# beyzoskaya/HiC-GNN

Hardware: AMD Instinct MI355X
Metric: training steps/sec (GATNetSelectiveResidualsUpdated, fwd+loss+bwd+Adam) (higher is better)
Workload: dtype fp32; 1 GPU; synth-20000; n_nodes=20000, nnz_with_self_loops=4019956, d=512, heads=2, loss=mse, parallelism=single, gemm=fp32 MFMA

## Files before the change

### hic-gnn_amd/csrc/gemm.hip

```cpp
#include <algorithm>
#include <cstdlib>

#include "reduce.hpp"

namespace hicgat {

typedef float f32x16 __attribute__((ext_vector_type(16)));

constexpr int GK = 16;

constexpr int kOcc64 = 6, kOcc128 = 1;

template <int BM, int BN, bool A_KM, bool B_KM, bool VEC, bool DB, bool CS = false>
__device__ __forceinline__ void gemm_tile(const float *__restrict__ A, int64_t lda,
                                          const float *__restrict__ B, int64_t ldb,
                                          float *__restrict__ C, int64_t ldc, int M, int N,
                                          int K, int kchunk, const float *__restrict__ bias,
                                          float *__restrict__ slab, int64_t slab_stride, int accumulate,
                                          float *__restrict__ csum, int bx, int by, int bz,
                                          float *__restrict__ crelu = nullptr, int64_t ldr = 0) {
  static_assert(!CS || A_KM, "column sums of A need the K-major (weight-gradient) layout");
  constexpr int WM = BM / 2, WN = BN / 2;
  constexpr int TM = WM / 32, TN = WN / 32;
  constexpr int AE = VEC ? BM * GK / 1024 : BM * GK / 256;
// ... 166 lines not shown
                                                   float *__restrict__ csum) {
  gemm_tile<BM, BN, A_KM, B_KM, VEC, DB, CS>(A, lda, B, ldb, C, ldc, M, N, K, kchunk, bias, slab, slab_stride, accumulate,
                                             csum, blockIdx.x, blockIdx.y, blockIdx.z);
}

__global__ void colsum_zero_kernel(float *out, int N, int accumulate) {
  const int n = blockIdx.x * 256 + threadIdx.x;
  if (n < N && !accumulate) out[n] = 0.f;
}

int gemm_wgrad_ring_launch(const float *A, int64_t lda, const float *B, int64_t ldb, int M, int N, int K, int kchunk,
                           int splits, float *slab, int64_t slab_stride, hipStream_t s);

template <int BM, int BN, bool AK, bool BK_>
static int launch(const float *A, int64_t lda, const float *B, int64_t ldb, float *C, int64_t ldc, int M, int N,
                  int K, int splits, const float *bias, float *slab, int acc, hipStream_t s, float *csum = nullptr,
                  bool ring = false) {
  const int kchunk = ((K + splits - 1) / splits + GK - 1) / GK * GK;
  const dim3 grid((M + BM - 1) / BM, (N + BN - 1) / BN, splits);
  const bool a_ok = AK ? (M % 4 == 0 && lda % 4 == 0) : (K % 4 == 0 && lda % 4 == 0);
  const bool b_ok = BK_ ? (N % 4 == 0 && ldb % 4 == 0) : (K % 4 == 0 && ldb % 4 == 0);
  const bool al = ((reinterpret_cast<uintptr_t>(A) | reinterpret_cast<uintptr_t>(B)) & 15) == 0;
  const bool cs = AK && csum != nullptr;
  const int64_t stride = (int64_t)M * N + (cs ? M : 0);
  float *sl = splits > 1 ? slab : nullptr;
  float *cdst = cs ? (sl ? slab + (int64_t)M * N : csum) : nullptr;
#define HICGAT_GEMM_GO(V, D, C_)                                                                            \
  hipLaunchKernelGGL((gemm_kernel<BM, BN, AK, BK_, V, D, C_>), grid, dim3(256), 0, s, A, lda, B, ldb, C, ldc, M, N, \
                     K, kchunk, bias, sl, stride, acc, cdst)
  int ring_rc = HICGAT_EUNSUPPORTED;
  if (ring && AK && BK_ && BM == 128 && BN == 128 && sl && !cs)
    ring_rc = gemm_wgrad_ring_launch(A, lda, B, ldb, M, N, K, kchunk, splits, sl, stride, s);
  if (ring_rc == HICGAT_OK) {
  } else if (ring_rc != HICGAT_EUNSUPPORTED) {
    return ring_rc;
  } else if (a_ok && b_ok && al) {
    constexpr bool db = !AK && BK_;
    if (cs) HICGAT_GEMM_GO(true, db, AK);
    else HICGAT_GEMM_GO(true, db, false);
  } else {
    if (cs) HICGAT_GEMM_GO(false, false, AK);
    else HICGAT_GEMM_GO(false, false, false);
  }
#undef HICGAT_GEMM_GO
  HICGAT_CHECK_LAUNCH();
  if (splits > 1) {
    const ColOut o{C, ldc, N, nullptr, bias, acc, cs ? csum : nullptr, (int64_t)M * N};
    return colsum_wide_launch(slab, stride, splits, stride, o, s);
  }
  return HICGAT_OK;
}

int gemm_tall_launch(bool b_kmajor, const float *A, int64_t lda, const float *B, int64_t ldb, float *C, int64_t ldc,
                     int M, int N, int K, const float *bias, int accumulate, hipStream_t s);

static int64_t tall_min_tiles() { return 192; }

template <bool AK, bool BK_>
static int dispatch(const float *A, int64_t lda, const float *B, int64_t ldb, float *C, int64_t ldc, int M, int N,
                    int K, int splits, const float *bias, float *slab, int acc, int impl, hipStream_t s) {
  if (!AK && splits == 1 && M >= 1024 &&
      (int64_t)((M + 159) / 160) * (N / 128) >= tall_min_tiles()) {
    const int rc = gemm_tall_launch(BK_, A, lda, B, ldb, C, ldc, M, N, K, bias, acc, s);
    if (rc != HICGAT_EUNSUPPORTED) return rc;
  }
  if (M >= 128 && N >= 128 && M <= 1024) {
    const bool ring = AK && BK_ && impl == HICGAT_GEMM_AUTO && splits > 1 && M % 128 == 0 && N % 128 == 0 &&
                      N <= 1024 && lda % 4 == 0 && ldb % 4 == 0;
    return launch<128, 128, AK, BK_>(A, lda, B, ldb, C, ldc, M, N, K, splits, bias, slab, acc, s, nullptr, ring);
  }
  if (N >= 128) return launch<64, 128, AK, BK_>(A, lda, B, ldb, C, ldc, M, N, K, splits, bias, slab, acc, s);
  return launch<64, 64, AK, BK_>(A, lda, B, ldb, C, ldc, M, N, K, splits, bias, slab, acc, s);
}

constexpr int kMaxWJobs = 16, kMaxCJobs = 32, kGroupTile = 128;
constexpr int64_t WEIGHTED_LG1_ROWS = 1024;
#ifndef HICGAT_COLSUM_SHORT
#define HICGAT_COLSUM_SHORT 16
#endif
constexpr int64_t kColsumShortRows = HICGAT_COLSUM_SHORT;
constexpr int kWeightedLg = 1;
template <int KMAX>
__device__ __forceinline__ int find_job(const int (&start)[KMAX], int n, int b) {
  int q = 0;
#pragma unroll
  for (int k = 1; k < KMAX; ++k) q += (k < n && b >= start[k]) ? 1 : 0;
  return q;
}
struct WJob {
  const float *dy;
  const float *x;
  float *dw;
  float *db;
  float *slab;
  int64_t ldy, ldx, lddw;
  int M, N, K, kchunk, tm, tn, wg0, accumulate, vec;
};
struct WJobs {
  int start[kMaxWJobs];
  WJob j[kMaxWJobs];
  int n;
};
__global__ __launch_bounds__(256, kOcc128) void wgrad_grouped_kernel(const WJobs jobs) {
  const int q = find_job(jobs.start, jobs.n, (int)blockIdx.x);
  const WJob &J = jobs.j[q];
  const int local = blockIdx.x - J.wg0, per = J.tm * J.tn;
  const int bz = local / per, rem = local - bz * per, bx = rem % J.tm, by = rem / J.tm;
  const int64_t stride = (int64_t)J.M * J.N + J.M;
  float *cs = J.db ? (J.slab ? J.slab + (int64_t)J.M * J.N : J.db) : nullptr;
  if (J.vec)
    gemm_tile<kGroupTile, kGroupTile, true, true, true, false, true>(J.dy, J.ldy, J.x, J.ldx, J.dw, J.lddw, J.M, J.N,
                                                                     J.K, J.kchunk, nullptr, J.slab, stride,
                                                                     J.accumulate, cs, bx, by, bz);
  else
    gemm_tile<kGroupTile, kGroupTile, true, true, false, false, true>(J.dy, J.ldy, J.x, J.ldx, J.dw, J.lddw, J.M, J.N,
                                                                      J.K, J.kchunk, nullptr, J.slab, stride,
// ... 301 lines not shown
    J.wg0 = wg;
    wj.start[wj.n - 1] = wg;
    wg += J.tm * J.tn * sp;
    if (sp > 1) {
      const int64_t stride = (int64_t)a.M * a.N + a.M;
      int rc = add_col(J.slab, stride, sp, (int64_t)a.M * a.N, a.dw, a.accumulate);
      if (rc != HICGAT_OK) return rc;
      if (a.db && (rc = add_col(J.slab + (int64_t)a.M * a.N, stride, sp, a.M, a.db, a.accumulate)) != HICGAT_OK)
        return rc;
    }
  }
  for (int i = 0; i < nc; ++i) {
    if (c[i].rows < 0 || c[i].cols < 0 || (c[i].cols > 0 && !c[i].dst) || (c[i].rows > 0 && !c[i].src))
      return HICGAT_EINVAL;
    const int rc = add_col(c[i].src, c[i].ld, c[i].rows, c[i].cols, c[i].dst, c[i].accumulate, c[i].wt, c[i].ldw,
                           c[i].segs, c[i].ldd);
    if (rc != HICGAT_OK) return rc;
  }
  if (wg > 0) {
    hipLaunchKernelGGL(wgrad_grouped_kernel, dim3(wg), dim3(256), 0, s, wj);
    HICGAT_CHECK_LAUNCH();
  }
  if (blk > 0) {
    hipLaunchKernelGGL(colsum_grouped_kernel, dim3(blk), dim3(256), 0, s, cj);
    HICGAT_CHECK_LAUNCH();
  }
  return HICGAT_OK;
}

extern "C" size_t hicgat_gemm_workspace_bytes(int M, int N, int splits) {
  return splits > 1 ? (size_t)splits * M * N * sizeof(float) : 0;
}

extern "C" int hicgat_gemm(int a_kmajor, int b_kmajor, int M, int N, int K, const float *A, int64_t lda,
                           const float *B, int64_t ldb, const float *bias, float *C, int64_t ldc,
                           int accumulate, int splits, int impl, void *workspace, size_t workspace_bytes,
                           hicgat_stream_t stream) {
  if (impl == HICGAT_GEMM_X3) return HICGAT_EUNSUPPORTED;
  if (impl != HICGAT_GEMM_AUTO && impl != HICGAT_GEMM_F32) return HICGAT_EINVAL;
  if (M < 0 || N < 0 || K < 0 || splits < 1) return HICGAT_EINVAL;
  if (M == 0 || N == 0) return HICGAT_OK;
  if (!A || !B || !C) return HICGAT_EINVAL;
  if (splits > 1 && (!workspace || workspace_bytes < hicgat_gemm_workspace_bytes(M, N, splits)))
    return HICGAT_EINVAL;
  hipStream_t s = (hipStream_t)stream;
  float *slab = static_cast<float *>(workspace);
  const int i = impl;
  if (!a_kmajor && !b_kmajor) return dispatch<false, false>(A, lda, B, ldb, C, ldc, M, N, K, splits, bias, slab, accumulate, i, s);
  if (!a_kmajor && b_kmajor) return dispatch<false, true>(A, lda, B, ldb, C, ldc, M, N, K, splits, bias, slab, accumulate, i, s);
  if (a_kmajor && !b_kmajor) return dispatch<true, false>(A, lda, B, ldb, C, ldc, M, N, K, splits, bias, slab, accumulate, i, s);
  return dispatch<true, true>(A, lda, B, ldb, C, ldc, M, N, K, splits, bias, slab, accumulate, i, s);
}

extern "C" size_t hicgat_gemm_wgrad_workspace_bytes(int M, int N, int splits) {
  return splits > 1 ? (size_t)splits * ((size_t)M * N + M) * sizeof(float) : 0;
}

extern "C" int hicgat_gemm_wgrad(int M, int N, int K, const float *dY, int64_t ldy, const float *X, int64_t ldx,
                                 float *dW, int64_t lddw, float *db, int accumulate, int splits, void *workspace,
                                 size_t workspace_bytes, hicgat_stream_t stream) {
  if (M < 0 || N < 0 || K < 0 || splits < 1 || lddw < N) return HICGAT_EINVAL;
  if (M == 0 || N == 0) return HICGAT_OK;
  if (!dY || !X || !dW) return HICGAT_EINVAL;
  if (splits > 1 && (!workspace || workspace_bytes < hicgat_gemm_wgrad_workspace_bytes(M, N, splits)))
    return HICGAT_EINVAL;
  hipStream_t s = (hipStream_t)stream;
  float *slab = static_cast<float *>(workspace);
  if (M >= 128 && N >= 128 && M <= 1024)
    return launch<128, 128, true, true>(dY, ldy, X, ldx, dW, lddw, M, N, K, splits, nullptr, slab, accumulate, s, db);
  if (N >= 128) return launch<64, 128, true, true>(dY, ldy, X, ldx, dW, lddw, M, N, K, splits, nullptr, slab, accumulate, s, db);
  return launch<64, 64, true, true>(dY, ldy, X, ldx, dW, lddw, M, N, K, splits, nullptr, slab, accumulate, s, db);
}

extern "C" size_t hicgat_colsum_workspace_bytes(int K, int N) { return colsum_workspace_bytes(K, N); }

extern "C" int hicgat_colsum(const float *A, int64_t lda, int K, int N, float *out, int accumulate, void *workspace,
                             size_t workspace_bytes, hicgat_stream_t stream) {
  if (K < 0 || N < 0) return HICGAT_EINVAL;
  if (N == 0) return HICGAT_OK;
  if (!out || (K > 0 && !A)) return HICGAT_EINVAL;
  const size_t need = colsum_workspace_bytes(K, N);
  if (need > 0 && (!workspace || workspace_bytes < need)) return HICGAT_EINVAL;
  hipStream_t s = (hipStream_t)stream;
  const ColOut o{out, 0, N, nullptr, nullptr, accumulate};
  if (K == 0) {
    hipLaunchKernelGGL(colsum_zero_kernel, dim3((N + 255) / 256), dim3(256), 0, s, out, N, accumulate);
    HICGAT_CHECK_LAUNCH();
    return HICGAT_OK;
  }
  return colsum_launch(A, lda, K, N, o, static_cast<float *>(workspace), s);
}
```

### hic-gnn_amd/csrc/gemm_tall.hip

```cpp
#include "common.hpp"

namespace hicgat {

namespace {

constexpr int TBM = 160, TBN = 128, TBK = 16, TSLOTS = 3;
constexpr int TA_F = TBM * TBK;
constexpr int TB_F = TBN * TBK;
constexpr int TSTAGE_F = TA_F + TB_F;
constexpr size_t kTallLds = (size_t)TSLOTS * TSTAGE_F * sizeof(float);
constexpr int TA_PIECES = TA_F * 4 / 1024;
constexpr int TB_PIECES = TB_F * 4 / 1024;

typedef float f32x16 __attribute__((ext_vector_type(16)));
typedef float f4v __attribute__((ext_vector_type(4)));

__device__ __forceinline__ int kc_slot(int r, int g) { return g ^ ((r >> 2) & 3); }

template <bool BKC>
__device__ __forceinline__ void tall_issue(float *stage, const float *__restrict__ A, int64_t lda, int m0, int M,
                                           const float *__restrict__ B, int64_t ldb, int n0, int k0, int w,
                                           int lane) {
  for (int p = w; p < TA_PIECES; p += 4) {
    const int r = 16 * p + (lane >> 2), s = lane & 3;
    const int gm = min(m0 + r, M - 1);
    const float *src = A + (size_t)gm * lda + k0 + 4 * kc_slot(r, s);
    __builtin_amdgcn_global_load_lds(src, stage + p * 256, 16, 0, 0);
  }
  float *bs = stage + TA_F;
  for (int p = w; p < TB_PIECES; p += 4) {
    const float *src;
    if (BKC) {
      const int r = 16 * p + (lane >> 2), s = lane & 3;
      src = B + (size_t)(n0 + r) * ldb + k0 + 4 * kc_slot(r, s);
    } else {
      const int t = 2 * p + (lane >> 5);
      src = B + (size_t)(k0 + t) * ldb + n0 + (lane & 31) * 4;
    }
    __builtin_amdgcn_global_load_lds(src, bs + p * 256, 16, 0, 0);
  }
}

}

template <bool BKC>
__global__ __launch_bounds__(256, 2) void gemm_tall_kernel(const float *__restrict__ A, int64_t lda,
                                                          const float *__restrict__ B, int64_t ldb,
                                                          float *__restrict__ C, int64_t ldc, int M, int N, int K,
                                                          const float *__restrict__ bias, int accumulate) {
  extern __shared__ __attribute__((aligned(16))) float lds[];
  const int lane = threadIdx.x & 63, w = wave_in_block();
  const int li = lane & 31, lk = lane >> 5;
  const int ntn = N / TBN;
  const int tile = xcd_remap(blockIdx.x, gridDim.x);
  const int m0 = (tile / ntn) * TBM, n0 = (tile % ntn) * TBN;
  const int S = K / TBK;
  f32x16 acc[5];
#pragma unroll
  for (int t = 0; t < 5; ++t)
#pragma unroll
    for (int r = 0; r < 16; ++r) acc[t][r] = 0.f;

  tall_issue<BKC>(lds, A, lda, m0, M, B, ldb, n0, 0, w, lane);
  if (S > 1) tall_issue<BKC>(lds + TSTAGE_F, A, lda, m0, M, B, ldb, n0, TBK, w, lane);
  const bool w_more = w < TA_PIECES - 8;

  const int bcol = 32 * w + li;
  const uint32_t lds_base = (uint32_t)(uintptr_t)lds;
  const uint32_t a_row = (uint32_t)(li * TBK * 4);
  const uint32_t b_row = (uint32_t)(TA_F * 4) + (BKC ? (uint32_t)(bcol * TBK * 4) : (uint32_t)(bcol * 4));

  for (int s = 0; s < S; ++s) {
    if (s + 1 < S) {
      if (w_more) asm volatile("s_waitcnt vmcnt(5)" ::: "memory");
      else asm volatile("s_waitcnt vmcnt(4)" ::: "memory");
    } else {
      asm volatile("s_waitcnt vmcnt(0)" ::: "memory");
    }
    asm volatile("s_waitcnt lgkmcnt(0)" ::: "memory");
    __builtin_amdgcn_s_barrier();
    asm volatile("" ::: "memory");
    if (s + 2 < S)
      tall_issue<BKC>(lds + ((s + 2) % TSLOTS) * TSTAGE_F, A, lda, m0, M, B, ldb, n0, (s + 2) * TBK, w, lane);
    const uint32_t st = lds_base + (uint32_t)((s % TSLOTS) * TSTAGE_F * 4);
#pragma unroll
    for (int p = 0; p < TBK / 8; ++p) {
      const int g = 2 * p + lk;
      const uint32_t aa = st + a_row + (uint32_t)(kc_slot(li, g) * 16);
      f4v a0, a1, a2, a3, a4;
      float bk[4];
      if (BKC) {
        const uint32_t ba = st + b_row + (uint32_t)(kc_slot(bcol, g) * 16);
        f4v b;
        asm volatile(
            "ds_read_b128 %0, %6\n\tds_read_b128 %1, %6 offset:2048\n\tds_read_b128 %2, %6 offset:4096\n\t"
            "ds_read_b128 %3, %6 offset:6144\n\tds_read_b128 %4, %6 offset:8192\n\tds_read_b128 %5, %7\n\t"
            "s_waitcnt lgkmcnt(0)"
            : "=&v"(a0), "=&v"(a1), "=&v"(a2), "=&v"(a3), "=&v"(a4), "=&v"(b)
            : "v"(aa), "v"(ba)
            : "memory");
        bk[0] = b.x;
        bk[1] = b.y;
        bk[2] = b.z;
        bk[3] = b.w;
      } else {
        const uint32_t ba = st + b_row + (uint32_t)((8 * p + 4 * lk) * TBN * 4);
        asm volatile(
            "ds_read_b128 %0, %9\n\tds_read_b128 %1, %9 offset:2048\n\tds_read_b128 %2, %9 offset:4096\n\t"
            "ds_read_b128 %3, %9 offset:6144\n\tds_read_b128 %4, %9 offset:8192\n\t"
            "ds_read_b32 %5, %10\n\tds_read_b32 %6, %10 offset:512\n\tds_read_b32 %7, %10 offset:1024\n\t"
            "ds_read_b32 %8, %10 offset:1536\n\ts_waitcnt lgkmcnt(0)"
            : "=&v"(a0), "=&v"(a1), "=&v"(a2), "=&v"(a3), "=&v"(a4), "=&v"(bk[0]), "=&v"(bk[1]), "=&v"(bk[2]), "=&v"(bk[3])
            : "v"(aa), "v"(ba)
            : "memory");
      }
      const f4v a[5] = {a0, a1, a2, a3, a4};
#pragma unroll
      for (int c = 0; c < 4; ++c)
#pragma unroll
        for (int t = 0; t < 5; ++t) acc[t] = __builtin_amdgcn_mfma_f32_32x32x2f32(a[t][c], bk[c], acc[t], 0, 0, 0);
    }
  }

  const int gn = n0 + bcol;
  const float bb = bias ? bias[gn] : 0.f;
#pragma unroll
  for (int t = 0; t < 5; ++t) {
    float old[16];
#pragma unroll
    for (int r = 0; r < 16; ++r) old[r] = 0.f;
    if (accumulate) {
#pragma unroll
      for (int r = 0; r < 16; ++r) {
        const int gm = min(m0 + 32 * t + (r & 3) + 8 * (r >> 2) + 4 * lk, M - 1);
        old[r] = C[(size_t)gm * ldc + gn];
      }
    }
#pragma unroll
    for (int r = 0; r < 16; ++r) {
      const int gm = m0 + 32 * t + (r & 3) + 8 * (r >> 2) + 4 * lk;
      if (gm < M) C[(size_t)gm * ldc + gn] = acc[t][r] + bb + old[r];
    }
  }
}

int gemm_tall_launch(bool b_kmajor, const float *A, int64_t lda, const float *B, int64_t ldb, float *C, int64_t ldc,
                     int M, int N, int K, const float *bias, int accumulate, hipStream_t s) {
  const bool al = ((reinterpret_cast<uintptr_t>(A) | reinterpret_cast<uintptr_t>(B)) & 15) == 0;
  if (!al || M < TBM || N % TBN || K % TBK || K < TBK || lda % 4 || ldb % 4) return HICGAT_EUNSUPPORTED;
  const int64_t tiles = (int64_t)((M + TBM - 1) / TBM) * (N / TBN);
  if (tiles > 0x7fffffff) return HICGAT_EUNSUPPORTED;
  if (b_kmajor)
    hipLaunchKernelGGL(gemm_tall_kernel<false>, dim3((unsigned)tiles), dim3(256), kTallLds, s, A, lda, B, ldb, C, ldc, M,
                       N, K, bias, accumulate);
  else
    hipLaunchKernelGGL(gemm_tall_kernel<true>, dim3((unsigned)tiles), dim3(256), kTallLds, s, A, lda, B, ldb, C, ldc, M,
                       N, K, bias, accumulate);
  HICGAT_CHECK_LAUNCH();
  return HICGAT_OK;
}

}
```

### hic-gnn_amd/hicgat/_lib.py

```python
import ctypes
import os

import torch

from . import streams as _streams

_HERE = os.path.dirname(os.path.abspath(__file__))
LIB_PATH = os.environ.get("HICGAT_LIB", os.path.join(_HERE, "libhicgat.so"))

c_int, c_i64, c_f, c_d, c_sz, c_p = (ctypes.c_int, ctypes.c_int64, ctypes.c_float, ctypes.c_double,
                                     ctypes.c_size_t, ctypes.c_void_p)
c_u64, c_u32 = ctypes.c_uint64, ctypes.c_uint32


class WgradJob(ctypes.Structure):
    _fields_ = [("dy", c_p), ("ldy", c_i64), ("x", c_p), ("ldx", c_i64), ("dw", c_p), ("lddw", c_i64), ("db", c_p),
                ("M", c_int), ("N", c_int), ("K", c_int), ("accumulate", c_int)]


class ColsumJob(ctypes.Structure):
    _fields_ = [("src", c_p), ("ld", c_i64), ("rows", c_i64), ("cols", c_i64), ("dst", c_p), ("accumulate", c_int),
                ("wt", c_p), ("ldw", c_i64), ("segs", c_int), ("ldd", c_i64)]


# ... 23 lines not shown
                                       c_i64, c_p, c_i64, c_p, c_p, c_f, c_p, c_p, c_int, c_p]),
    "hicgat_gat_agg_drop_fwd": (c_int, [c_p, c_p, c_int, c_int, c_int, c_int, c_int, c_int, c_p, c_p, c_p,
                                        c_p, c_f, c_int, c_p, c_p, c_p, c_d, c_u64, c_p, c_i64, c_u32, c_p]),
    "hicgat_gat_agg_drop_bwd_src": (c_int, [c_p, c_p, c_int, c_int, c_int, c_int, c_int, c_p, c_p, c_p, c_p,
                                            c_i64, c_p, c_i64, c_p, c_p, c_f, c_p, c_p, c_int, c_d, c_u64, c_p,
                                            c_i64, c_u32, c_p]),
    "hicgat_gat_attn_mask": (c_int, [c_p, c_p, c_int, c_int, c_d, c_u64, c_p, c_i64, c_u32, c_p, c_p]),
    "hicgat_gat_agg_fwd_tiled": (c_int, [c_p, c_p, c_p, c_p, c_p, c_p, c_p, c_int, c_int, c_int, c_int, c_int,
                                         c_int, c_p, c_p, c_p, c_p, c_f, c_int, c_p, c_p, c_p, c_int, c_p, c_sz,
                                         c_p]),
    "hicgat_gat_agg_bwd_src_tiled": (c_int, [c_p, c_p, c_p, c_p, c_p, c_int, c_int, c_int, c_int, c_int, c_int,
                                             c_p, c_p, c_p, c_p, c_i64, c_p, c_i64, c_p, c_p, c_f, c_p, c_p, c_int,
                                             c_p, c_sz, c_p]),
    "hicgat_gat_tiled_workspace_bytes": (c_sz, [c_int, c_int]),
    "hicgat_gat_param_grad": (c_int, [c_p, c_p, c_p, c_p, c_int, c_int, c_int, c_p, c_p, c_p, c_int, c_p,
                                      c_sz, c_p]),
    "hicgat_gat_param_grad_workspace_bytes": (c_sz, [c_int, c_int]),
    "hicgat_gat_transpose_map": (c_int, [c_p, c_p, c_int, c_p, c_p]),
    "hicgat_gat_alpha": (c_int, [c_p, c_p, c_int, c_int, c_int, c_p, c_p, c_p, c_f, c_p, c_p]),
    "hicgat_gat_alpha_bwd_dst": (c_int, [c_p, c_p, c_int, c_int, c_int, c_p, c_p, c_p, c_p, c_f, c_p, c_p, c_p]),
    "hicgat_gat_alpha_bwd_src": (c_int, [c_p, c_p, c_p, c_int, c_int, c_int, c_p, c_p, c_p, c_p, c_p, c_p, c_p, c_p,
                                         c_f, c_p, c_p, c_p, c_p]),
    "hicgat_pairdist_fwd": (c_int, [c_p, c_int, c_p, c_i64, c_p]),
    "hicgat_pairdist_bwd": (c_int, [c_p, c_p, c_int, c_i64, c_p, c_p, c_sz, c_p]),
    "hicgat_pairdist_mse_fused": (c_int, [c_p, c_p, c_int, c_i64, c_i64, c_i64, c_i64, c_i64, c_i64, c_int,
                                          c_p, c_p, c_p, c_p, c_sz, c_p]),
    "hicgat_pairdist_finalize": (c_int, [c_int, c_int, c_p, c_p, c_p]),
    "hicgat_pairdist_finalize_rows": (c_int, [c_int, c_int, c_p, c_p, c_p, c_int, c_int, c_p, c_p, c_p, c_p, c_p]),
    "hicgat_pairdist_num_tiles": (c_i64, [c_int, c_int]),
    "hicgat_pairdist_workspace_bytes": (c_sz, [c_int, c_int]),
    "hicgat_pairdist_mse_fused_support": (c_int, [c_p, c_p, c_int, c_f, c_p, c_p, c_p, c_p, c_i64, c_i64,
                                                  c_int, c_int, c_int, c_p, c_p, c_p, c_p, c_p, c_sz, c_p]),
    "hicgat_pairdist_support_workspace_bytes": (c_sz, [c_int]),
    "hicgat_xagg_vec_bytes": (c_sz, []),
    "hicgat_xagg_logits": (c_int, [c_p, c_p, c_p, c_p, c_int, c_int, c_int, c_int, c_p, c_p, c_p, c_p,
                                   c_i64, c_p, c_p, c_p, c_p, c_sz, c_p]),
    "hicgat_xagg_fwd": (c_int, [c_p, c_p, c_int, c_int, c_int, c_int, c_int, c_int, c_p, c_p, c_p, c_f, c_p, c_p,
                                c_p]),
    "hicgat_xagg_bias_relu": (c_int, [c_p, c_p, c_p, c_int, c_int, c_p]),
    "hicgat_xagg_rows_bwd": (c_int, [c_int, c_int, c_int, c_p, c_p, c_p, c_p, c_p, c_p]),
    "hicgat_xagg_edge": (c_int, [c_p, c_p, c_int, c_int, c_int, c_int, c_int, c_int, c_p, c_p, c_p, c_p, c_p, c_p,
                                 c_f, c_p, c_p]),
    "hicgat_xagg_edge_acc": (c_int, [c_p, c_p, c_int, c_int, c_int, c_int, c_int, c_int, c_p, c_p, c_p, c_p, c_p,
                                     c_p, c_f, c_p, c_p]),
    "hicgat_xagg_edge_acc_blocks": (c_int, [c_int]),
    "hicgat_xagg_slab_workspace_bytes": (c_sz, []),
    "hicgat_xagg_slab_sum": (c_int, [c_p, c_p, c_int, c_p, c_p, c_p, c_p, c_p, c_sz, c_p]),
    "hicgat_xagg_param_finish": (c_int, [c_p, c_p, c_p, c_p, c_p, c_int, c_i64, c_int, c_int, c_int, c_p, c_p,
                                         c_p, c_p]),
    "hicgat_truth_support": (c_int, [c_p, c_int, c_i64, c_f, c_p, c_p, c_p, c_p, c_p]),
    "hicgat_gemm": (c_int, [c_int, c_int, c_int, c_int, c_int, c_p, c_i64, c_p, c_i64, c_p, c_p, c_i64, c_int,
                            c_int, c_int, c_p, c_sz, c_p]),
    "hicgat_gemm_workspace_bytes": (c_sz, [c_int, c_int, c_int]),
    "hicgat_gemm_wgrad": (c_int, [c_int, c_int, c_int, c_p, c_i64, c_p, c_i64, c_p, c_i64, c_p, c_int, c_int, c_p,
                                  c_sz, c_p]),
    "hicgat_gemm_wgrad_workspace_bytes": (c_sz, [c_int, c_int, c_int]),
    "hicgat_gemm_rows_grouped_workspace_bytes": (c_sz, [c_gjobs, c_int, c_int]),
    "hicgat_gemm_rows_grouped": (c_int, [c_gjobs, c_int, c_int, c_int, c_p, c_sz, c_p]),
    "hicgat_param_grads_workspace_bytes": (c_sz, [c_wjobs, c_int, c_int]),
    "hicgat_param_grads_grouped": (c_int, [c_wjobs, c_int, c_cjobs, c_int, c_int, c_p, c_sz, c_p]),
    "hicgat_colsum": (c_int, [c_p, c_i64, c_int, c_int, c_p, c_int, c_p, c_sz, c_p]),
    "hicgat_colsum_workspace_bytes": (c_sz, [c_int, c_int]),
    "hicgat_ln_act_res_fwd": (c_int, [c_p, c_i64, c_int, c_int, c_p, c_p, c_f, c_int, c_f, c_p, c_i64, c_p, c_p, c_f,
                                      c_p, c_i64, c_p, c_p, c_p]),
    "hicgat_ln_act_res_bwd": (c_int, [c_p, c_i64, c_p, c_i64, c_int, c_int, c_p, c_p, c_p, c_int, c_f, c_p, c_i64,
                                      c_p, c_p, c_p, c_i64, c_p, c_i64, c_p, c_p, c_p, c_p, c_int, c_p, c_sz, c_p]),
    "hicgat_ln_act_res_bwd_params": (c_int, [c_int, c_p, c_p, c_p, c_p, c_int, c_p, c_sz, c_p]),
    "hicgat_ln_act_res_workspace_bytes": (c_sz, [c_int, c_int]),
    "hicgat_act_fwd": (c_int, [c_p, c_int, c_int, c_int, c_f, c_p, c_p]),
    "hicgat_act_bwd": (c_int, [c_p, c_p, c_int, c_int, c_int, c_f, c_p, c_p]),
    "hicgat_tail_pack_bytes": (c_sz, []),
    "hicgat_tail_pack": (c_int, [c_p, c_p, c_p, c_p, c_sz, c_p]),
    "hicgat_tail_fwd_fused": (c_int, [c_p, c_i64, c_int] + [c_p] * 14 + [c_f] + [c_p] * 10 + [c_p, c_p]),
    "hicgat_tail_bwd_waves": (c_int, []),
    "hicgat_tail_bwd_workspace_bytes": (c_sz, [c_int, c_int]),
    "hicgat_tail_bwd_fused": (c_int, [c_p, c_int] + [c_p] * 16 + [c_p] * 4 + [c_p, c_sz] * 3 + [c_p, c_p]),
    "hicgat_tail_fwd_fused_heads": (c_int, [c_p, c_i64, c_i64, c_p, c_p, c_p, c_p, c_int] + [c_p] * 14 + [c_f]
                                    + [c_p] * 10 + [c_p, c_p]),
    "hicgat_tail_bwd_fused_rows": (c_int, [c_p, c_int] + [c_p] * 16 + [c_p] * 3 + [c_p, c_sz] * 3
                                   + [c_int, c_p, c_p, c_p, c_p, c_p, c_p, c_p]),
    "hicgat_tail_bwd_fused_heads": (c_int, [c_p, c_int] + [c_p] * 16 + [c_p] * 3 + [c_p, c_sz] * 3
                                    + [c_int, c_p, c_p, c_p, c_p, c_p, c_p, c_p, c_p]),
    "hicgat_sage_weights": (c_int, [c_p, c_int, c_i64, c_p, c_p, c_p, c_p, c_p]),
    "hicgat_sage_agg": (c_int, [c_p, c_p, c_p, c_p, c_int, c_int, c_int, c_int, c_p, c_int, c_int, c_p, c_i64,
                                c_p]),
    "hicgat_kr_matvec": (c_int, [c_p, c_i64, c_int, c_p, c_p, c_p, c_p, c_p]),
    "hicgat_kr_scale": (c_int, [c_p, c_i64, c_int, c_p, c_p, c_i64, c_p]),
    "hicgat_n2v_walks": (c_int, [c_p, c_p, c_p, c_int, c_p, c_int, c_int, c_f, c_f, c_u64, c_p, c_p]),
    "hicgat_n2v_sgns_epoch": (c_int, [c_p, c_int, c_int, c_p, c_p, c_int, c_int, c_int, c_int, c_f, c_f, c_int,
                                      c_int, c_u64, c_int, c_p, c_p, c_p]),
    "hicgat_line_workspace_bytes": (c_sz, [c_int, c_int]),
    "hicgat_line_samples": (c_int, [c_p, c_p, c_p, c_p, c_int, c_p, c_p, c_int, c_p, c_i64, c_i64, c_int, c_int,
                                    c_u64, c_i64, c_i64, c_p, c_p, c_p, c_p]),
    "hicgat_line_train": (c_int, [c_p, c_p, c_p, c_p, c_int, c_p, c_p, c_int, c_p, c_i64, c_i64, c_int, c_int, c_int,
                                  c_u64, c_i64, c_i64, c_d, c_d, c_d, c_d, c_p, c_p, c_p, c_p, c_p, c_p, c_p, c_sz,
                                  c_p]),
    "hicgat_adam_step": (c_int, [c_p, c_p, c_p, c_p, c_i64, c_d, c_d, c_d, c_d, c_i64, c_p]),
    "hicgat_adam_step_table": (c_int, [c_p, c_p, c_p, c_p, c_i64, c_d, c_d, c_d, c_p, c_i64, c_p, c_int, c_p]),
    "hicgat_step_begin": (c_int, [c_p, c_i64, c_p, c_p]),
    "hicgat_step_begin_pack": (c_int, [c_p, c_i64, c_p, c_p, c_p, c_p, c_p, c_sz, c_p]),
    "hicgat_act_dropout_fwd": (c_int, [c_p, c_i64, c_int, c_int, c_int, c_f, c_d, c_u64, c_p, c_i64, c_u32, c_i64,
                                       c_p, c_i64, c_p]),
    "hicgat_act_dropout_bwd": (c_int, [c_p, c_i64, c_p, c_i64, c_int, c_int, c_int, c_f, c_d, c_p, c_i64, c_p]),
    "hicgat_dropout_mask": (c_int, [c_p, c_int, c_int, c_d, c_u64, c_p, c_i64, c_u32, c_i64, c_p]),
    "hicgat_dropout_advance": (c_int, [c_p, c_p]),
    "hicgat_bn_workspace_bytes": (c_sz, [c_int, c_int]),
# ... 70 lines not shown
```

### hic-gnn_amd/hicgat/kernels.py

```python
import os

import torch

from . import _lib
from .paramgrads import ColsumJob, WeightGradJob

TIMERS = None
GEMM_AUTO = 0
GEMM_F32 = 1


class _timed:
    def __init__(self, name):
        self.name = name

    def __enter__(self):
        if TIMERS is not None:
            self.e0 = torch.cuda.Event(enable_timing=True)
            self.e0.record()

    def __exit__(self, *a):
        if TIMERS is not None:
            e1 = torch.cuda.Event(enable_timing=True)
            e1.record()
# ... 324 lines not shown
    def fused_loss_support_range(self, coords, sf, n, kind, t0, t1, s0, s1, stats, loss, dcoords, cmap=None):
        ws = _lib.workspace(self.lib.hicgat_pairdist_support_workspace_bytes(n), coords.device)
        d32, d64 = (None, dcoords) if dcoords.dtype == torch.float64 else (dcoords, None)
        assert cmap is None or (cmap.dtype == torch.int32 and cmap.numel() == n)
        with _timed("pairdist_mse_fused"):
            _lib.check(self.lib.hicgat_pairdist_mse_fused_support(
                P(coords), P(cmap), n, sf.background, P(sf.rowptr), P(sf.col_buf), P(sf.val_buf), P(sf.diag), int(t0),
                int(t1), int(s0), int(s1), int(kind), P(stats), P(loss), P(d32), P(d64), P(ws), ws.numel(),
                _lib.stream(coords.device)), "hicgat_pairdist_mse_fused_support")

    def loss_finalize(self, n, kind, stats, loss, dc64=None, r0=0, r1=0, dcoords=None, reorder=None):
        if dc64 is None:
            _lib.check(self.lib.hicgat_pairdist_finalize(n, int(kind), P(stats), P(loss), _lib.stream(stats.device)),
                       "hicgat_pairdist_finalize")
            return
        assert dc64.is_contiguous() and dcoords.is_contiguous() and dc64.shape == dcoords.shape == (n, 3)
        cbuf, gidx, cglob = reorder if reorder is not None else (None, None, None)
        if reorder is not None:
            assert cbuf.is_contiguous() and cglob.shape == (n, 3) and gidx.dtype == torch.int32 and gidx.numel() == n
        _lib.check(self.lib.hicgat_pairdist_finalize_rows(n, int(kind), P(stats), P(loss), P(dc64), int(r0), int(r1),
                                                          P(dcoords), P(cbuf), P(gidx), P(cglob),
                                                          _lib.stream(stats.device)),
                   "hicgat_pairdist_finalize_rows")

    def pairdist_fwd(self, coords):
        n = coords.shape[0]
        D = torch.empty((n, n), dtype=torch.float32, device=coords.device)
        _lib.check(self.lib.hicgat_pairdist_fwd(P(coords), n, P(D), n, _lib.stream(coords.device)),
                   "hicgat_pairdist_fwd")
        return D

    def pairdist_bwd(self, coords, G):
        n = coords.shape[0]
        dc = torch.empty_like(coords)
        ws = _lib.workspace(self.lib.hicgat_pairdist_workspace_bytes(n, self.PD_SQUARE), coords.device)
        _lib.check(self.lib.hicgat_pairdist_bwd(P(coords), P(G), n, G.shape[1], P(dc), P(ws), ws.numel(),
                                                _lib.stream(coords.device)), "hicgat_pairdist_bwd")
        return dc

    def gemm(self, a_kmajor, b_kmajor, M, N, K, A, B, C, bias=None, accumulate=False, splits=None, name="gemm",
             impl=None):
        dev = C.device
        ws = None
        impl = self.gemm_impl if impl is None else impl
        if splits is None:
            splits = row_splits(M, N, K) if (not a_kmajor and impl in (GEMM_AUTO, GEMM_F32)) else 1
        if splits > 1:
            ws = _lib.workspace(self.lib.hicgat_gemm_workspace_bytes(M, N, splits), dev)
        with _timed(name):
            _lib.check(self.lib.hicgat_gemm(int(a_kmajor), int(b_kmajor), M, N, K, P(A), A.stride(0), P(B),
                                            B.stride(0), P(bias), P(C), C.stride(0), int(accumulate), int(splits),
                                            int(impl), P(ws), 0 if ws is None else ws.numel(), _lib.stream(dev)),
                       "hicgat_gemm")
        return C

    def wgrad(self, dy, x, W_out, b_out=None, accumulate=False, splits=1):
        K_, M = dy.shape
        N = x.shape[1]
        dev = W_out.device
        ws = None
        if splits > 1:
            ws = _lib.workspace(self.lib.hicgat_gemm_wgrad_workspace_bytes(M, N, splits), dev)
        with _timed("gemm_dw"):
            _lib.check(self.lib.hicgat_gemm_wgrad(M, N, K_, P(dy), dy.stride(0), P(x), x.stride(0), P(W_out),
                                                  W_out.stride(0), P(b_out), int(accumulate), int(splits), P(ws),
                                                  0 if ws is None else ws.numel(), _lib.stream(dev)),
                       "hicgat_gemm_wgrad")
        return W_out, b_out

    GROUP_WGS = int(os.environ.get("HICGAT_GROUP_WGS", "512"))
    ROWS_WGS = int(os.environ.get("HICGAT_ROWS_WGS", "512"))
    SMALL_M = 16

    def param_grads_grouped(self, wjobs, cjobs, target_wgs=None, small_m=None):
        target = self.GROUP_WGS if target_wgs is None else target_wgs
        small_m = self.SMALL_M if small_m is None else small_m
        big, cjobs = [], [ColsumJob(*j) for j in cjobs]
        for j in (WeightGradJob(*j) for j in wjobs):
            if j.dy.shape[1] < small_m:
                cjobs += [ColsumJob(j.x, j.dW[m], j.accumulate, j.dy[:, m]) for m in range(j.dy.shape[1])]
                if j.db is not None:
                    cjobs.append(ColsumJob(j.dy, j.db, j.accumulate))
            else:
                big.append(j)
        wjobs = big
        W = (_lib.WgradJob * max(1, len(wjobs)))()
        for k, (dy, x, dw, db, acc) in enumerate(wjobs):
            assert dy.stride(1) == 1 and x.stride(1) == 1 and dw.stride(1) == 1 and dy.shape[0] == x.shape[0]
            assert db is None or db.is_contiguous()
            W[k] = _lib.WgradJob(dy.data_ptr(), dy.stride(0), x.data_ptr(), x.stride(0), dw.data_ptr(), dw.stride(0),
                                 None if db is None else db.data_ptr(), dy.shape[1], x.shape[1], dy.shape[0], int(acc))
        C = (_lib.ColsumJob * max(1, len(cjobs)))()
        for k, (src, dst, acc, wt) in enumerate(cjobs):
            assert src.dim() == 2 and src.stride(1) == 1
            if dst.dim() == 2:
                assert dst.stride(1) == 1 and dst.shape[1] == src.shape[1] and 1 <= dst.shape[0] <= max(1, src.shape[0])
                segs, ldd = dst.shape[0], dst.stride(0)
            else:
                assert dst.is_contiguous() and dst.numel() == src.shape[1]
                segs, ldd = 1, 0
            assert wt is None or (wt.dim() == 1 and wt.shape[0] == src.shape[0])
            C[k] = _lib.ColsumJob(src.data_ptr(), src.stride(0), src.shape[0], src.shape[1], dst.data_ptr(), int(acc),
                                  None if wt is None else wt.data_ptr(), 0 if wt is None else wt.stride(0), segs, ldd)
        dev = (wjobs[0][0] if wjobs else cjobs[0][0]).device
        ws = _lib.workspace(self.lib.hicgat_param_grads_workspace_bytes(W, len(wjobs), target), dev)
        with _timed("param_grads_grouped"):
# ... 274 lines not shown
```

### include/hicgat.h

```cpp
#ifndef HICGAT_H
#define HICGAT_H

#include <stddef.h>
#include <stdint.h>

#ifdef __cplusplus
extern "C" {
#endif

typedef void *hicgat_stream_t;

enum { HICGAT_LOSS_MSE = 0, HICGAT_LOSS_COMBINED = 1, HICGAT_LOSS_CONTRASTIVE = 2 };

enum {
  HICGAT_OK = 0,
  HICGAT_EINVAL = -1,
  HICGAT_ELAUNCH = -2,
  HICGAT_EUNSUPPORTED = -3
};

int hicgat_version(void);
const char *hicgat_strerror(int code);

int hicgat_csr_from_dense(const double *A, int N, int64_t lda, int32_t *rowptr, int32_t *col,
// ... 86 lines not shown

int hicgat_gat_agg_fwd_tiled(const int32_t *rowptr, const int32_t *col, const int32_t *rowptr_s,
                             const int32_t *col_s, const int32_t *tptr, const int32_t *tcol,
                             const uint32_t *tmask, int ntiles, int N, int H, int C, int row_begin,
                             int row_end, const float *h, const float *a_src, const float *a_dst,
                             const float *bias, float neg_slope, int act, float *out, float *out2,
                             float *row_stats, int splits, void *workspace, size_t workspace_bytes,
                             hicgat_stream_t stream);
int hicgat_gat_agg_bwd_src_tiled(const int32_t *rowptr_s, const int32_t *col_s, const int32_t *tptr,
                                 const int32_t *tcol, const uint32_t *tmask, int ntiles, int N, int H,
                                 int C, int row_begin, int row_end, const float *h, const float *a_src,
                                 const float *a_dst, const float *row_stats, int64_t ld_stats,
                                 const float *dout, int64_t ld_dout, const float *att_src,
                                 const float *att_dst, float neg_slope, float *dh, float *da_src,
                                 int splits, void *workspace, size_t workspace_bytes,
                                 hicgat_stream_t stream);
size_t hicgat_gat_tiled_workspace_bytes(int rows, int splits);
int hicgat_gat_param_grad(const float *h, const float *dout, const float *da_src,
                          const float *row_stats, int N, int H, int C, float *datt_src,
                          float *datt_dst, float *dbias, int accumulate, void *workspace,
                          size_t workspace_bytes, hicgat_stream_t stream);
size_t hicgat_gat_param_grad_workspace_bytes(int N, int D);

int hicgat_pairdist_fwd(const float *coords, int N, float *D, int64_t ldd, hicgat_stream_t stream);
int hicgat_pairdist_bwd(const float *coords, const float *G, int N, int64_t ldg, float *dcoords,
                        void *workspace, size_t workspace_bytes, hicgat_stream_t stream);

int hicgat_pairdist_mse_fused(const float *coords, const float *T, int N, int64_t ldt, int64_t t_row0,
                              int64_t t_rows, int64_t t_col0, int64_t tile_begin, int64_t tile_end,
                              int loss_kind, double *stats, float *loss, float *dcoords, void *workspace,
                              size_t workspace_bytes, hicgat_stream_t stream);
int hicgat_pairdist_finalize(int N, int loss_kind, double *stats, float *loss, hicgat_stream_t stream);
int hicgat_pairdist_finalize_rows(int N, int loss_kind, double *stats, float *loss, const double *dc64,
                                  int row_begin, int row_end, float *dcoords, const float *cbuf,
                                  const int32_t *gidx, float *cglob, hicgat_stream_t stream);
enum { HICGAT_PD_SQUARE = 0, HICGAT_PD_TRI = 1 };
int64_t hicgat_pairdist_num_tiles(int N, int mode);
size_t hicgat_pairdist_workspace_bytes(int N, int mode);
int hicgat_pairdist_mse_fused_support(const float *coords, const int32_t *cmap, int N, float background,
                                      const int32_t *rowptr, const int32_t *col, const float *val,
                                      const float *diag, int64_t tile_begin, int64_t tile_end,
                                      int support_row_begin, int support_row_end, int loss_kind,
                                      double *stats, float *loss, float *dcoords, double *dcoords64,
                                      void *workspace, size_t workspace_bytes, hicgat_stream_t stream);
size_t hicgat_pairdist_support_workspace_bytes(int N);
int hicgat_truth_support(const float *T, int N, int64_t ldt, float background, int32_t *rowptr, int32_t *col,
                         float *val, float *diag, hicgat_stream_t stream);

enum { HICGAT_GEMM_AUTO = 0, HICGAT_GEMM_F32 = 1, HICGAT_GEMM_X3 = 2 };
int hicgat_gemm(int a_kmajor, int b_kmajor, int M, int N, int K, const float *A, int64_t lda,
                const float *B, int64_t ldb, const float *bias, float *C, int64_t ldc, int accumulate,
                int splits, int impl, void *workspace, size_t workspace_bytes, hicgat_stream_t stream);
size_t hicgat_gemm_workspace_bytes(int M, int N, int splits);
int hicgat_gemm_wgrad(int M, int N, int K, const float *dY, int64_t ldy, const float *X, int64_t ldx, float *dW,
                      int64_t lddw, float *db, int accumulate, int splits, void *workspace, size_t workspace_bytes,
                      hicgat_stream_t stream);
size_t hicgat_gemm_wgrad_workspace_bytes(int M, int N, int splits);
typedef struct hicgat_wgrad_job {
  const float *dy;
  int64_t ldy;
  const float *x;
  int64_t ldx;
  float *dw;
  int64_t lddw;
  float *db;
  int M, N, K, accumulate;
} hicgat_wgrad_job;
typedef struct hicgat_colsum_job {
  const float *src;
  int64_t ld;
  int64_t rows;
  int64_t cols;
  float *dst;
  int accumulate;
  const float *wt;
  int64_t ldw;
  int segs;
  int64_t ldd;
} hicgat_colsum_job;
size_t hicgat_param_grads_workspace_bytes(const hicgat_wgrad_job *wjobs, int nw, int target_wgs);
int hicgat_param_grads_grouped(const hicgat_wgrad_job *wjobs, int nw, const hicgat_colsum_job *cjobs, int nc,
                               int target_wgs, void *workspace, size_t workspace_bytes, hicgat_stream_t stream);
typedef struct hicgat_gemm_job {
  const float *a;
  int64_t lda;
  const float *b;
  int64_t ldb;
  float *c;
  int64_t ldc;
  float *c_relu;
  int64_t ldr;
  const float *bias;
  int M, N, K;
} hicgat_gemm_job;
size_t hicgat_gemm_rows_grouped_workspace_bytes(const hicgat_gemm_job *jobs, int n, int splits);
int hicgat_gemm_rows_grouped(const hicgat_gemm_job *jobs, int n, int b_kmajor, int splits, void *workspace,
                             size_t workspace_bytes, hicgat_stream_t stream);
int hicgat_colsum(const float *A, int64_t lda, int K, int N, float *out, int accumulate, void *workspace,
                  size_t workspace_bytes, hicgat_stream_t stream);
size_t hicgat_colsum_workspace_bytes(int K, int N);

int hicgat_ln_act_res_fwd(const float *y, int64_t ldy, int M, int W, const float *gamma, const float *beta, float eps,
                          int act, float slope, const float *res, int64_t ldr, const float *gamma2, const float *beta2,
                          float eps2, float *z, int64_t ldz, float *row_stats, float *row_stats2,
                          hicgat_stream_t stream);
int hicgat_ln_act_res_bwd(const float *dz, int64_t lddz, const float *y, int64_t ldy, int M, int W,
// ... 139 lines not shown
```

Baseline: 593.1 steps/s.

## Add software-pipelined tall GEMM kernel with interleaved async LDS loads and MFMA

Adds a new tall-GEMM kernel that rotates through a three-slot LDS ring. Each wave issues global_load_lds copies through inline asm that sets m0, and hand-scheduled ds_read_b128 fragment reads interleave with the 32x32x2 fp32 MFMAs, so global loads, LDS reads and math overlap within each K step. The old kernel is kept as the 'burst' variant and is used only when impl is F32; AUTO now takes the new path. The change also exposes a direct hicgat_gemm_tall entry point and factors out the store epilogue. The hand-written asm waitcnt and barrier scheduling is fragile: a wrong count would race on LDS. The new kernel is launched with zero dynamic LDS and uses a static shared array instead.

```diff
diff --git a/hic-gnn_amd/csrc/gemm.hip b/hic-gnn_amd/csrc/gemm.hip
--- a/hic-gnn_amd/csrc/gemm.hip
+++ b/hic-gnn_amd/csrc/gemm.hip
@@ -242,7 +242,8 @@
 }
 
 int gemm_tall_launch(bool b_kmajor, const float *A, int64_t lda, const float *B, int64_t ldb, float *C, int64_t ldc,
-                     int M, int N, int K, const float *bias, int accumulate, hipStream_t s);
+                     int M, int N, int K, const float *bias, int accumulate, bool burst,
+                     hipStream_t s);
 
 static int64_t tall_min_tiles() { return 192; }
 
@@ -251,7 +252,7 @@
                     int K, int splits, const float *bias, float *slab, int acc, int impl, hipStream_t s) {
   if (!AK && splits == 1 && M >= 1024 &&
       (int64_t)((M + 159) / 160) * (N / 128) >= tall_min_tiles()) {
-    const int rc = gemm_tall_launch(BK_, A, lda, B, ldb, C, ldc, M, N, K, bias, acc, s);
+    const int rc = gemm_tall_launch(BK_, A, lda, B, ldb, C, ldc, M, N, K, bias, acc, impl == HICGAT_GEMM_F32, s);
     if (rc != HICGAT_EUNSUPPORTED) return rc;
   }
   if (M >= 128 && N >= 128 && M <= 1024) {
@@ -659,6 +660,17 @@
   return dispatch<true, true>(A, lda, B, ldb, C, ldc, M, N, K, splits, bias, slab, accumulate, i, s);
 }
 
+extern "C" int hicgat_gemm_tall(int b_kmajor, int M, int N, int K, const float *A, int64_t lda, const float *B,
+                                int64_t ldb, const float *bias, float *C, int64_t ldc, int accumulate, int impl,
+                                hicgat_stream_t stream) {
+  if (impl != HICGAT_GEMM_AUTO && impl != HICGAT_GEMM_F32) return HICGAT_EINVAL;
+  if (M < 0 || N < 0 || K < 0 || lda < K || ldb < (b_kmajor ? N : K) || ldc < N) return HICGAT_EINVAL;
+  if (M == 0 || N == 0) return HICGAT_OK;
+  if (!A || !B || !C) return HICGAT_EINVAL;
+  return gemm_tall_launch(b_kmajor != 0, A, lda, B, ldb, C, ldc, M, N, K, bias, accumulate, impl == HICGAT_GEMM_F32,
+                          (hipStream_t)stream);
+}
+
 extern "C" size_t hicgat_gemm_wgrad_workspace_bytes(int M, int N, int splits) {
   return splits > 1 ? (size_t)splits * ((size_t)M * N + M) * sizeof(float) : 0;
 }
diff --git a/hic-gnn_amd/csrc/gemm_tall.hip b/hic-gnn_amd/csrc/gemm_tall.hip
--- a/hic-gnn_amd/csrc/gemm_tall.hip
+++ b/hic-gnn_amd/csrc/gemm_tall.hip
@@ -9,6 +9,7 @@
 constexpr int TB_F = TBN * TBK;
 constexpr int TSTAGE_F = TA_F + TB_F;
 constexpr size_t kTallLds = (size_t)TSLOTS * TSTAGE_F * sizeof(float);
+static_assert(kTallLds <= 80 * 1024, "two workgroups per CU in 160 KiB of LDS");
 constexpr int TA_PIECES = TA_F * 4 / 1024;
 constexpr int TB_PIECES = TB_F * 4 / 1024;
 
@@ -41,10 +42,41 @@
   }
 }
 
+__device__ __forceinline__ void tall_glds(const float *src, uint32_t dst) {
+  uint32_t keep;
+  asm volatile("s_mov_b32 %0, m0\n\ts_mov_b32 m0, %2\n\ts_nop 0\n\tglobal_load_lds_dwordx4 %1, off\n\ts_mov_b32 m0, %0"
+               : "=&s"(keep)
+               : "v"(src), "s"(dst)
+               : "memory");
+}
+
+__device__ __forceinline__ void tall_store(const f32x16 (&acc)[5], float *__restrict__ C, int64_t ldc, int M, int m0,
+                                           int gn, int lk, const float *__restrict__ bias, int accumulate) {
+  const float bb = bias ? bias[gn] : 0.f;
+#pragma unroll
+  for (int t = 0; t < 5; ++t) {
+    float old[16];
+#pragma unroll
+    for (int r = 0; r < 16; ++r) old[r] = 0.f;
+    if (accumulate) {
+#pragma unroll
+      for (int r = 0; r < 16; ++r) {
+        const int gm = min(m0 + 32 * t + (r & 3) + 8 * (r >> 2) + 4 * lk, M - 1);
+        old[r] = C[(size_t)gm * ldc + gn];
+      }
+    }
+#pragma unroll
+    for (int r = 0; r < 16; ++r) {
+      const int gm = m0 + 32 * t + (r & 3) + 8 * (r >> 2) + 4 * lk;
+      if (gm < M) C[(size_t)gm * ldc + gn] = acc[t][r] + bb + old[r];
+    }
+  }
+}
+
 }
 
 template <bool BKC>
-__global__ __launch_bounds__(256, 2) void gemm_tall_kernel(const float *__restrict__ A, int64_t lda,
+__global__ __launch_bounds__(256, 2) void gemm_tall_burst_kernel(const float *__restrict__ A, int64_t lda,
                                                           const float *__restrict__ B, int64_t ldb,
                                                           float *__restrict__ C, int64_t ldc, int M, int N, int K,
                                                           const float *__restrict__ bias, int accumulate) {
@@ -122,40 +154,181 @@
     }
   }
 
-  const int gn = n0 + bcol;
-  const float bb = bias ? bias[gn] : 0.f;
-#pragma unroll
-  for (int t = 0; t < 5; ++t) {
-    float old[16];
-#pragma unroll
-    for (int r = 0; r < 16; ++r) old[r] = 0.f;
-    if (accumulate) {
-#pragma unroll
-      for (int r = 0; r < 16; ++r) {
-        const int gm = min(m0 + 32 * t + (r & 3) + 8 * (r >> 2) + 4 * lk, M - 1);
-        old[r] = C[(size_t)gm * ldc + gn];
+  tall_store(acc, C, ldc, M, m0, n0 + bcol, lk, bias, accumulate);
+}
+
+template <bool BKC>
+__global__ __launch_bounds__(256, 2) void gemm_tall_kernel(const float *__restrict__ A, int64_t lda,
+                                                          const float *__restrict__ B, int64_t ldb,
+                                                          float *__restrict__ C, int64_t ldc, int M, int N, int K,
+                                                          const float *__restrict__ bias, int accumulate) {
+  static_assert(TBK == 16, "two k-group pairs per stage: one per fragment register set");
+  __shared__ __attribute__((aligned(16))) float lds[TSLOTS * TSTAGE_F];
+  const int lane = threadIdx.x & 63, w = wave_in_block();
+  const int li = lane & 31, lk = lane >> 5;
+  const int ntn = N / TBN;
+  const int tile = xcd_remap(blockIdx.x, gridDim.x);
+  const int m0 = (tile / ntn) * TBM, n0 = (tile % ntn) * TBN;
+  const int S = K / TBK;
+  f32x16 acc[5];
+#pragma unroll
+  for (int t = 0; t < 5; ++t)
+#pragma unroll
+    for (int r = 0; r < 16; ++r) acc[t][r] = 0.f;
+
+  const bool w_more = w < TA_PIECES - 8;
+  const float *pa[3], *pb[2];
+#pragma unroll
+  for (int h = 0; h < 3; ++h) {
+    const int r = 16 * (w + 4 * h) + (lane >> 2);
+    pa[h] = A + (size_t)min(m0 + r, M - 1) * lda + 4 * kc_slot(r, lane & 3);
+  }
+#pragma unroll
+  for (int h = 0; h < 2; ++h) {
+    const int p = w + 4 * h;
+    if (BKC) {
+      const int r = 16 * p + (lane >> 2);
+      pb[h] = B + (size_t)(n0 + r) * ldb + 4 * kc_slot(r, lane & 3);
+    } else {
+      pb[h] = B + (size_t)(2 * p + (lane >> 5)) * ldb + n0 + (lane & 31) * 4;
+    }
+  }
+  const int64_t b_step = BKC ? (int64_t)TBK : (int64_t)TBK * ldb;
+  const uint32_t lds_base = (uint32_t)(uintptr_t)lds;
+  auto issue = [&](int slot_, int q) {
+    const uint32_t dst = lds_base + (uint32_t)((slot_ * TSTAGE_F + (q & 1) * TA_F + (w + 4 * (q >> 1)) * 256) * 4);
+    tall_glds((q & 1) ? pb[q >> 1] : pa[q >> 1], dst);
+  };
+  auto advance = [&](int q, bool more) {
+    if (q & 1) pb[q >> 1] += more ? b_step : (int64_t)0;
+    else pa[q >> 1] += more ? TBK : 0;
+  };
+#pragma unroll
+  for (int st = 0; st < 2; ++st) {
+#pragma unroll
+    for (int q = 0; q < 4; ++q) issue(st, q);
+    if (w_more) issue(st, 4);
+#pragma unroll
+    for (int q = 0; q < 5; ++q) advance(q, st + 1 < S);
+  }
+
+  const int bcol = 32 * w + li;
+  uint32_t a_off[2], b_off[2];
+#pragma unroll
+  for (int p = 0; p < 2; ++p) {
+    a_off[p] = (uint32_t)(li * TBK * 4 + kc_slot(li, 2 * p + lk) * 16);
+    b_off[p] = (uint32_t)(TA_F * 4) + (BKC ? (uint32_t)(bcol * TBK * 4 + kc_slot(bcol, 2 * p + lk) * 16)
+                                           : (uint32_t)(bcol * 4 + (8 * p + 4 * lk) * TBN * 4));
+  }
+
+  f4v fa[2][5], fb[2];
+  float fs[2][4];
+  auto read = [&](int x, uint32_t aa, uint32_t ba) {
+    if constexpr (BKC) {
+      asm volatile(
+          "ds_read_b128 %0, %6\n\tds_read_b128 %1, %6 offset:2048\n\tds_read_b128 %2, %6 offset:4096\n\t"
+          "ds_read_b128 %3, %6 offset:6144\n\tds_read_b128 %4, %6 offset:8192\n\tds_read_b128 %5, %7"
+          : "=&v"(fa[x][0]), "=&v"(fa[x][1]), "=&v"(fa[x][2]), "=&v"(fa[x][3]), "=&v"(fa[x][4]), "=&v"(fb[x])
+          : "v"(aa), "v"(ba)
+          : "memory");
+    } else {
+      asm volatile(
+          "ds_read_b128 %0, %9\n\tds_read_b128 %1, %9 offset:2048\n\tds_read_b128 %2, %9 offset:4096\n\t"
+          "ds_read_b128 %3, %9 offset:6144\n\tds_read_b128 %4, %9 offset:8192\n\t"
+          "ds_read_b32 %5, %10\n\tds_read_b32 %6, %10 offset:512\n\tds_read_b32 %7, %10 offset:1024\n\t"
+          "ds_read_b32 %8, %10 offset:1536"
+          : "=&v"(fa[x][0]), "=&v"(fa[x][1]), "=&v"(fa[x][2]), "=&v"(fa[x][3]), "=&v"(fa[x][4]), "=&v"(fs[x][0]),
+            "=&v"(fs[x][1]), "=&v"(fs[x][2]), "=&v"(fs[x][3])
+          : "v"(aa), "v"(ba)
+          : "memory");
+    }
+  };
+#define TALL_LANDED(x, behind)                                                                                       \
+  do {                                                                                                               \
+    if constexpr (BKC)                                                                                               \
+      asm volatile("s_waitcnt lgkmcnt(" #behind ")"                                                                  \
+                   : "+v"(fa[x][0]), "+v"(fa[x][1]), "+v"(fa[x][2]), "+v"(fa[x][3]), "+v"(fa[x][4]), "+v"(fb[x])     \
+                   :                                                                                                 \
+                   : "memory");                                                                                      \
+    else                                                                                                             \
+      asm volatile("s_waitcnt lgkmcnt(" #behind ")"                                                                  \
+                   : "+v"(fa[x][0]), "+v"(fa[x][1]), "+v"(fa[x][2]), "+v"(fa[x][3]), "+v"(fa[x][4]), "+v"(fs[x][0]), \
+                     "+v"(fs[x][1]), "+v"(fs[x][2]), "+v"(fs[x][3])                                                  \
+                   :                                                                                                 \
+                   : "memory");                                                                                      \
+  } while (0)
+  auto mma = [&](int x, auto between) {
+#pragma unroll
+    for (int i = 0; i < 20; ++i) {
+      const int c = i / 5, t = i % 5;
+      acc[t] = __builtin_amdgcn_mfma_f32_32x32x2f32(fa[x][t][c], BKC ? fb[x][c] : fs[x][c], acc[t], 0, 0, 0);
+      between(i);
+    }
+  };
+
+  if (w_more) asm volatile("s_waitcnt vmcnt(5)" ::: "memory");
+  else asm volatile("s_waitcnt vmcnt(4)" ::: "memory");
+  __builtin_amdgcn_s_barrier();
+  asm volatile("" ::: "memory");
+  read(0, lds_base + a_off[0], lds_base + b_off[0]);
+
+  int slot = 0;
+  for (int s = 0; s < S; ++s) {
+    const uint32_t st = lds_base + (uint32_t)(slot * TSTAGE_F * 4);
+    const int nslot = slot == 0 ? TSLOTS - 1 : slot - 1;
+    const int slot1 = slot == TSLOTS - 1 ? 0 : slot + 1;
+    const bool more = s + 3 < S;
+    read(1, st + a_off[1], st + b_off[1]);
+    if constexpr (BKC) TALL_LANDED(0, 6);
+    else TALL_LANDED(0, 9);
+    __builtin_amdgcn_sched_barrier(0);
+    mma(0, [&](int i) {
+      if (i == 2 || i == 11) {
+        const int q = i == 2 ? 0 : 1;
+        __builtin_amdgcn_sched_barrier(0);
+        issue(nslot, q);
+        advance(q, more);
+        __builtin_amdgcn_sched_barrier(0);
       }
-    }
-#pragma unroll
-    for (int r = 0; r < 16; ++r) {
-      const int gm = m0 + 32 * t + (r & 3) + 8 * (r >> 2) + 4 * lk;
-      if (gm < M) C[(size_t)gm * ldc + gn] = acc[t][r] + bb + old[r];
-    }
-  }
+    });
+    __builtin_amdgcn_sched_barrier(0);
+    TALL_LANDED(1, 0);
+    if (s + 1 < S) {
+      asm volatile("s_waitcnt vmcnt(2)" ::: "memory");
+      __builtin_amdgcn_s_barrier();
+      asm volatile("" ::: "memory");
+      const uint32_t sn = lds_base + (uint32_t)(slot1 * TSTAGE_F * 4);
+      read(0, sn + a_off[0], sn + b_off[0]);
+    }
+    __builtin_amdgcn_sched_barrier(0);
+    mma(1, [&](int i) {
+      if (i == 2 || i == 8 || i == 14) {
+        const int q = i == 2 ? 2 : i == 8 ? 3 : 4;
+        __builtin_amdgcn_sched_barrier(0);
+        if (q < 4 || w_more) issue(nslot, q);
+        advance(q, more);
+        __builtin_amdgcn_sched_barrier(0);
+      }
+    });
+    __builtin_amdgcn_sched_barrier(0);
+    slot = slot1;
+  }
+#undef TALL_LANDED
+  asm volatile("s_waitcnt vmcnt(0)" ::: "memory");
+
+  tall_store(acc, C, ldc, M, m0, n0 + bcol, lk, bias, accumulate);
 }
 
 int gemm_tall_launch(bool b_kmajor, const float *A, int64_t lda, const float *B, int64_t ldb, float *C, int64_t ldc,
-                     int M, int N, int K, const float *bias, int accumulate, hipStream_t s) {
+                     int M, int N, int K, const float *bias, int accumulate, bool burst, hipStream_t s) {
   const bool al = ((reinterpret_cast<uintptr_t>(A) | reinterpret_cast<uintptr_t>(B)) & 15) == 0;
   if (!al || M < TBM || N % TBN || K % TBK || K < TBK || lda % 4 || ldb % 4) return HICGAT_EUNSUPPORTED;
   const int64_t tiles = (int64_t)((M + TBM - 1) / TBM) * (N / TBN);
   if (tiles > 0x7fffffff) return HICGAT_EUNSUPPORTED;
-  if (b_kmajor)
-    hipLaunchKernelGGL(gemm_tall_kernel<false>, dim3((unsigned)tiles), dim3(256), kTallLds, s, A, lda, B, ldb, C, ldc, M,
-                       N, K, bias, accumulate);
-  else
-    hipLaunchKernelGGL(gemm_tall_kernel<true>, dim3((unsigned)tiles), dim3(256), kTallLds, s, A, lda, B, ldb, C, ldc, M,
-                       N, K, bias, accumulate);
+  auto *kernel = b_kmajor ? (burst ? gemm_tall_burst_kernel<false> : gemm_tall_kernel<false>)
+                          : (burst ? gemm_tall_burst_kernel<true> : gemm_tall_kernel<true>);
+  hipLaunchKernelGGL(kernel, dim3((unsigned)tiles), dim3(256), burst ? kTallLds : 0, s, A, lda, B, ldb, C, ldc, M, N, K, bias,
+                     accumulate);
   HICGAT_CHECK_LAUNCH();
   return HICGAT_OK;
 }
diff --git a/hic-gnn_amd/hicgat/_lib.py b/hic-gnn_amd/hicgat/_lib.py
--- a/hic-gnn_amd/hicgat/_lib.py
+++ b/hic-gnn_amd/hicgat/_lib.py
@@ -99,6 +99,8 @@
     "hicgat_gemm": (c_int, [c_int, c_int, c_int, c_int, c_int, c_p, c_i64, c_p, c_i64, c_p, c_p, c_i64, c_int,
                             c_int, c_int, c_p, c_sz, c_p]),
     "hicgat_gemm_workspace_bytes": (c_sz, [c_int, c_int, c_int]),
+    "hicgat_gemm_tall": (c_int, [c_int, c_int, c_int, c_int, c_p, c_i64, c_p, c_i64, c_p, c_p, c_i64, c_int, c_int,
+                                 c_p]),
     "hicgat_gemm_wgrad": (c_int, [c_int, c_int, c_int, c_p, c_i64, c_p, c_i64, c_p, c_i64, c_p, c_int, c_int, c_p,
                                   c_sz, c_p]),
     "hicgat_gemm_wgrad_workspace_bytes": (c_sz, [c_int, c_int, c_int]),
diff --git a/hic-gnn_amd/hicgat/kernels.py b/hic-gnn_amd/hicgat/kernels.py
--- a/hic-gnn_amd/hicgat/kernels.py
+++ b/hic-gnn_amd/hicgat/kernels.py
@@ -400,6 +400,12 @@
                                             B.stride(0), P(bias), P(C), C.stride(0), int(accumulate), int(splits),
                                             int(impl), P(ws), 0 if ws is None else ws.numel(), _lib.stream(dev)),
                        "hicgat_gemm")
+        return C
+
+    def gemm_tall(self, b_kmajor, M, N, K, A, B, C, bias=None, accumulate=False, impl=GEMM_AUTO):
+        _lib.check(self.lib.hicgat_gemm_tall(int(b_kmajor), M, N, K, P(A), A.stride(0), P(B), B.stride(0), P(bias),
+                                             P(C), C.stride(0), int(accumulate), int(impl), _lib.stream(C.device)),
+                   "hicgat_gemm_tall")
         return C
 
     def wgrad(self, dy, x, W_out, b_out=None, accumulate=False, splits=1):
diff --git a/include/hicgat.h b/include/hicgat.h
--- a/include/hicgat.h
+++ b/include/hicgat.h
@@ -162,6 +162,8 @@
                 const float *B, int64_t ldb, const float *bias, float *C, int64_t ldc, int accumulate,
                 int splits, int impl, void *workspace, size_t workspace_bytes, hicgat_stream_t stream);
 size_t hicgat_gemm_workspace_bytes(int M, int N, int splits);
+int hicgat_gemm_tall(int b_kmajor, int M, int N, int K, const float *A, int64_t lda, const float *B, int64_t ldb,
+                     const float *bias, float *C, int64_t ldc, int accumulate, int impl, hicgat_stream_t stream);
 int hicgat_gemm_wgrad(int M, int N, int K, const float *dY, int64_t ldy, const float *X, int64_t ldx, float *dW,
                       int64_t lddw, float *db, int accumulate, int splits, void *workspace, size_t workspace_bytes,
                       hicgat_stream_t stream);
```

Result: no change. 595.3 steps/s, median of 6 (+0.4%).
